# nsdumont/Semantic-Spiking-Neural-SLAM-2023

Hardware: AMD Instinct MI355X
Metric: sim-sec/wall-sec, SSP-SLAM ssp_dim=1015 10k PI neurons, 1/2/4/8 MI355X (higher is better)
Workload: dtype f32; 1 GPU; PathIntegration 2-D ssp_dim=1015 pi_n_neurons=10000/VCO (508 VCOs, 5080000 LIF neurons), configs[1]; eval_points_per_vco=4000, parallelism=1 GPU, build_cache=miss

## Files before the change

semantic-spiking-neural-slam-2023_amd/csrc/ssn_block.hpp:

```cpp
#pragma once
#include <type_traits>
#include "ssn_launch.hpp"

namespace ssn {

__device__ inline float wave_sum_dpp(float v) {
  int x;
#define SSN_DPP_ADD(ctrl, rmask)                                                                             \
  x = __builtin_amdgcn_update_dpp(0, __builtin_bit_cast(int, v), ctrl, rmask, 0xF, false);                    \
  v += __builtin_bit_cast(float, x);
  SSN_DPP_ADD(0xB1, 0xF)
  SSN_DPP_ADD(0x4E, 0xF)
  SSN_DPP_ADD(0x141, 0xF)
  SSN_DPP_ADD(0x140, 0xF)
  SSN_DPP_ADD(0x142, 0xA)
  SSN_DPP_ADD(0x143, 0xC)
#undef SSN_DPP_ADD
  return v;
}
__device__ inline float row_sum_dpp(float v) {
  int x;
#define SSN_DPP_ADD(ctrl)                                                                                    \
  x = __builtin_amdgcn_update_dpp(0, __builtin_bit_cast(int, v), ctrl, 0xF, 0xF, false);                      \
  v += __builtin_bit_cast(float, x);
// ... 124 lines not shown
  const f32x2 Wn = pk_fma_clamp01_vs_negv(spk, big, U);
  w = __builtin_elementwise_fma(spk, nu, Wn + nmt);
}
__device__ inline void lif_finish_silent(f32x2& w, f32x2 U, f32x2 nmt) {
  f32x2 Wn;
  asm("v_pk_mul_f32 %0, %1, -1.0 op_sel_hi:[1,0] clamp" : "=v"(Wn) : "v"(U));
  w = Wn + nmt;
}
__device__ inline f32x2 lif_input_part(f32x2 Jm1, f32x2& w, f32x2 W0, f32x2 em, const LifConstV3P& c, f32x2 big) {
  const f32x2 nmt = pk_sub_clamp01(w, (f32x2)(c.m1));
  const f32x2 U = __builtin_elementwise_fma(Jm1 + W0, em, -W0);
  const f32x2 spk = pk_mul_clamp01(U, big);
  f32x2 rc;
  rc.x = __builtin_amdgcn_rcpf(Jm1.x);
  rc.y = __builtin_amdgcn_rcpf(Jm1.y);
  f32x2 Wn, u, P, nu;
  asm("v_pk_fma_f32 %0, %2, %3, %4 neg_lo:[0,0,1] neg_hi:[0,0,1] clamp\n\t"
      "v_pk_mul_f32 %1, %4, %5"
      : "=&v"(Wn), "=v"(u)
      : "v"(spk), "s"(big), "v"(U), "v"(rc));
  asm("v_pk_fma_f32 %0, %1, %2, %3" : "=v"(P) : "v"(u), "v"((f32x2)(c.p2)), "s"((f32x2)(c.p1)));
  asm("v_pk_fma_f32 %0, %1, %2, %3" : "=v"(P) : "v"(u), "v"(P), "s"((f32x2)(c.p0)));
  asm("v_pk_fma_f32 %0, %1, %2, %3 clamp" : "=v"(nu) : "v"(u), "v"(P), "s"((f32x2)(c.ktau_ref)));
  w = __builtin_elementwise_fma(spk, nu, Wn + nmt);
  return spk;
}
__device__ inline float lif_word_in(float s, float K) { return __builtin_fmaf(-s, s < 0.0f ? K : 1.0f, 1.0f); }
__device__ inline float lif_word_out(float w, float K) { return (1.0f - w) * (w > 1.0f ? 1.0f / K : 1.0f); }

__device__ inline float bits_f(unsigned int x) { return __builtin_bit_cast(float, x); }
__device__ inline unsigned int f_bits(float x) { return __builtin_bit_cast(unsigned int, x); }

#ifdef SSN_BLOCK_STAMPS
__device__ unsigned long long g_block_stamps[9];
inline hipError_t read_block_stamps(unsigned long long* out, int reset) {
  hipError_t e = hipMemcpyFromSymbol(out, HIP_SYMBOL(g_block_stamps), sizeof(unsigned long long) * 9);
  if (e == hipSuccess && reset) {
    const unsigned long long z[9] = {0, 0, 0, 0, 0, 0, 0, 0, 0};
    e = hipMemcpyToSymbol(HIP_SYMBOL(g_block_stamps), z, sizeof z);
  }
  return e;
}
#define SSN_BSTAMP(var)                                                                          \
  do {                                                                                           \
    __builtin_amdgcn_sched_barrier(0);                                                           \
    asm volatile("s_memtime %0\n\ts_waitcnt lgkmcnt(0)" : "=s"(var) :: "memory");                \
    __builtin_amdgcn_sched_barrier(0);                                                           \
  } while (0)
#define SSN_BSTAMP_ADD(i, a, b) bst[i] += (b) - (a)
#else
#define SSN_BSTAMP(var) do {} while (0)
#define SSN_BSTAMP_ADD(i, a, b) do {} while (0)
#endif

#ifndef SSN_BLOCK_SKIP
#define SSN_BLOCK_SKIP 0
#endif
#ifndef SSN_BLOCK_PIPE
#define SSN_BLOCK_PIPE 1
#endif
#ifndef SSN_BLOCK_HOIST_A
#define SSN_BLOCK_HOIST_A 2
#endif
#ifndef SSN_BLOCK_HOIST_B
#define SSN_BLOCK_HOIST_B 4
#endif
#ifndef SSN_BLOCK_HOIST_C
#define SSN_BLOCK_HOIST_C 2
#endif
struct BlockHoist { int a, b, c; };
constexpr BlockHoist block_hoist(bool pipe, int tpb, int ng) {
  if (!pipe || SSN_BLOCK_SKIP != 0) return {0, 0, 0};
  const int room = tpb <= 512 && ng >= 10 ? ng : 0;
  const int c = SSN_BLOCK_HOIST_C >= 2 && room >= 2 ? 2 : 0;
  int b = SSN_BLOCK_HOIST_B < room - c ? SSN_BLOCK_HOIST_B : room - c;
  int a_ = SSN_BLOCK_HOIST_A < room - c - b ? SSN_BLOCK_HOIST_A : room - c - b;
  return {a_, b, c};
}

template <typename T, int DIN, int DOUT, int NPT, int TPB, int LDSW, int SPLIT = 0, int TAP = 0>
__global__ __launch_bounds__(TPB) void k_ens_block(BlockArgs<T> a) {
  static_assert(!(SPLIT && TAP), "the split kernel has no tapped form");
  constexpr bool ENC_LDS = LDSW == DIN;
  static_assert(LDSW == 0 || LDSW == DIN, "LDSW");
  extern __shared__ __align__(16) unsigned char ssn_block_dyn[];
  T* const e_lds = reinterpret_cast<T*>(ssn_block_dyn);
  constexpr bool F32 = sizeof(T) == 4;
  constexpr int PK = F32 ? 2 : 1;
  constexpr int NG = NPT / PK;
  static_assert(NPT % PK == 0, "f32 variants handle neuron pairs");
  constexpr bool PIPE = F32 && NG >= 5 && SSN_BLOCK_PIPE != 0;
  constexpr BlockHoist HO = block_hoist(PIPE, TPB, NG);
  constexpr int HC = HO.c, HA = HO.a, HB = HO.b, HT = HC + HA + HB;
  using G = typename std::conditional<F32, f32x2, T>::type;
  constexpr int DP = DOUT <= 4 ? 4 : 8;
  static_assert(!SPLIT || (sizeof(T) == 4 && DOUT <= 4), "split ensembles: f32, at most four decoded rows");
  const int P = SPLIT ? a.P : 1;
  const int k = P > 1 ? (int)blockIdx.x / P : (int)blockIdx.x;
  const int member = P > 1 ? (int)blockIdx.x - k * P : 0;
  const int noff = member * a.n_member;
  const int n_loc = P > 1 ? max(0, min(a.n_member, a.n_pad - noff)) : a.n_pad;
  const int tid = threadIdx.x;
  const int nthr = NG == 1 ? (int)blockDim.x : TPB;
  const int lane = tid & 63, wave = tid >> 6;
  const size_t row = (size_t)a.n_pad;
  const T* __restrict__ enc = a.enc + (size_t)k * DIN * row + noff;
  const T* __restrict__ bias = a.bias + (size_t)k * row + noff;
  T* __restrict__ Sp = a.S + (size_t)k * row + noff;
  const NeuronParams<T> np = a.np;
  const LifMath<T> lm(np);
  const int* tcol = nullptr;
  if constexpr (TAP != 0) {
    const int tslot = a.tap_slot[k];
    if (tslot >= 0) tcol = a.tap_col + (size_t)tslot * row;
// ... 18 lines not shown
    return reinterpret_cast<const G*>(e_lds + lrow[d] + g * nthr * PK);
  };
#pragma unroll
  for (int g = 0; g < NG; ++g) {
    const int i0 = (g * nthr + tid) * PK;
    const bool in = i0 < n_loc;
    const int ii = in ? i0 : 0;
    const T msk = in ? T(1) : T(0);
    auto ld = [&](const T* p) -> G { if constexpr (F32) return *reinterpret_cast<const f32x2*>(p) * msk; else return *p * msk; };
#pragma unroll
    for (int d = 0; d < DIN; ++d) {
      const G ev = ld(enc + d * row + ii);
      if constexpr (ENC_LDS) *reinterpret_cast<G*>(e_lds + d * cap + i0) = ev; else e[g][d] = ev;
    }
    b[g] = ld(bias + ii);
    s[g] = ld(Sp + ii);
    if constexpr (F32) {
      b[g] = b[g] - 1.0f;
      s[g] = (f32x2){lif_word_in(s[g].x, lcK), lif_word_in(s[g].y, lcK)};
    }
    if (a.dec_neuron_major) {
      const T* dp = a.dec + ((size_t)k * row + noff + ii) * DP;
#pragma unroll
      for (int r = 0; r < DOUT; ++r) {
        if constexpr (F32) dc[g][r] = (f32x2){dp[r], dp[DP + r]} * msk; else dc[g][r] = dp[r] * msk;
      }
    } else {
      const T* dp = a.dec + (size_t)k * DOUT * row + noff + ii;
#pragma unroll
      for (int r = 0; r < DOUT; ++r) dc[g][r] = ld(dp + r * row);
    }
  }

  constexpr int CH = 32;
  constexpr int XP = 4;
  constexpr int RW = DOUT <= 4 ? 64 : 128;
  __shared__ __align__(16) T red[2][RW];
  __shared__ __align__(16) T xs[CH][XP];
  __shared__ T os[CH][DOUT];
  __shared__ int s_dst[DOUT];
  __shared__ int s_out[DOUT];
  for (int i = tid; i < 2 * RW; i += nthr) (&red[0][0])[i] = T(0);
  if (tid < DOUT) { s_dst[tid] = a.didx[(long long)k * DOUT + tid]; s_out[tid] = a.rowout[(long long)k * DOUT + tid] ? 1 : 0; }
  const T* __restrict__ xbase = a.xrows + (size_t)a.row0 * a.n_sig + a.x_off + (long long)k * DIN;

  T fs[F32 ? 1 : DOUT], la[F32 ? 1 : DOUT], lb[F32 ? 1 : DOUT], tot[F32 ? 1 : DOUT];
  float F0 = 0.0f, F1 = 0.0f, la0 = 0.0f, lb0 = 0.0f, la1 = 0.0f, lb1 = 0.0f, v0 = 0.0f, v1 = 0.0f;
  T xa[DIN];
  int xr[DIN];
#pragma unroll
  for (int d = 0; d < DIN; ++d) {
    xr[d] = a.xrow[(long long)k * DIN + d];
    xa[d] = xr[d] >= 0 ? a.xalpha[(long long)k * DIN + d] : T(0);
  }
  if constexpr (F32) {
    const int r0 = lane >> 4;
    if (r0 < DOUT) {
      const long long i = (long long)k * DOUT + r0;
      const int st = a.lp_state[i];
      if (st >= 0) { F0 = a.sig[st]; la0 = a.lp_a[i]; lb0 = a.lp_b[i]; }
    }
    if (DOUT > 4) {
      const long long i = (long long)k * DOUT + 4;
      const int st = a.lp_state[i];
      if (st >= 0) { F1 = a.sig[st]; la1 = a.lp_a[i]; lb1 = a.lp_b[i]; }
    }
  } else {
#pragma unroll
    for (int r = 0; r < DOUT; ++r) {
      const long long i = (long long)k * DOUT + r;
      const int st = a.lp_state[i];
      fs[r] = st >= 0 ? a.sig[st] : T(0);
      la[r] = st >= 0 ? a.lp_a[i] : T(0);
      lb[r] = st >= 0 ? a.lp_b[i] : T(0);
// ... 13 lines not shown
  G en[ILE][LDSW > 0 ? LDSW : 1];
  if constexpr (ENC_LDS) {
#pragma unroll
    for (int u = 0; u < ILE; ++u)
#pragma unroll
      for (int d = 0; d < LDSW; ++d) en[u][d] = *lds_group(d, u);
  }
#ifdef SSN_BLOCK_STAMPS
  unsigned long long bst[6] = {0, 0, 0, 0, 0, 0}, bt0 = 0, bt1 = 0, bt2 = 0, bt3 = 0, bt4 = 0, bt5 = 0, bt6 = 0, bm0 = 0, br0 = 0;
  asm volatile("s_memtime %0\n\ts_memrealtime %1\n\ts_waitcnt lgkmcnt(0)" : "=s"(bm0), "=s"(br0) :: "memory");
#endif
  unsigned int n_slots = 0, n_silent = 0;
  T x[DIN];
  int xl[DIN];
#pragma unroll
  for (int d = 0; d < DIN; ++d) xl[d] = __builtin_amdgcn_readfirstlane((xr[d] & 3) << 4);
  auto assemble_x = [&](const float4 xv) {
    const float xin[4] = {xv.x, xv.y, xv.z, xv.w};
    float f1 = 0.0f;
    if constexpr (DOUT > 4) f1 = bits_f(__builtin_amdgcn_readlane(f_bits(F1), 0));
#pragma unroll
    for (int d = 0; d < DIN; ++d) {
      const float f0 = bits_f(__builtin_amdgcn_readlane(f_bits(F0), xl[d]));
      float st = f0;
      if constexpr (DOUT > 4) st = xr[d] >= 4 ? f1 : f0;
      x[d] = __builtin_fmaf(xa[d], st, xin[d]);
    }
  };
  f32x2 W0h[HT > 0 ? HT : 1], emh[HT > 0 ? HT : 1];
  if constexpr (HT > 0) {
#pragma unroll
    for (int g = 0; g < HT; ++g) lif_state_part(s[g], lc, W0h[g], emh[g]);
  }
  for (int j0 = 0; j0 < a.B; j0 += CH) {
    const int cn = min(CH, a.B - j0);
    __syncthreads();
    if (j0 > 0 && member == 0) {
      for (int i = tid; i < CH * DOUT; i += nthr) {
        const int jj = i / DOUT, r = i - jj * DOUT;
        if (s_out[r]) a.bsig[(size_t)(a.row0 + j0 - CH + jj) * a.n_sig + s_dst[r]] = os[jj][r];
      }
    }
    for (int i = tid; i < cn * DIN; i += nthr) {
      const int jj = i / DIN, d = i - jj * DIN;
      xs[jj][d] = xbase[(size_t)(j0 + jj) * a.n_sig + d];
    }
    __syncthreads();
    if constexpr (PIPE) {
      assemble_x(*(const float4*)xs[0]);
    }

    for (int jj = 0; jj < cn; ++jj) {
      SSN_BSTAMP(bt0);
      if constexpr (SPLIT != 0) {
        if (P > 1 && wave == 0 && (lane & 15) == 0) {
          unsigned int* const rst = a.xslots + (size_t)k * 64 + (size_t)((j0 + jj + 1) % 3) * ((size_t)a.K * 64) + member * 4 + (lane >> 4);
          const unsigned int sent = BLOCK_XCHG_SENTINEL;
          asm volatile("global_store_dword %0, %1, off sc0 sc1" :: "v"(rst), "v"(sent) : "memory");
        }
      }
      if constexpr (PIPE) {
      } else if constexpr (F32) {
        assemble_x(*(const float4*)xs[jj]);
      } else {
        T xin[XP];
        *(double2*)xin = *(const double2*)xs[jj]; *(double2*)(xin + 2) = *(const double2*)(xs[jj] + 2);
#pragma unroll
        for (int d = 0; d < DIN; ++d) {
          T st = T(0);
#pragma unroll
          for (int r = 0; r < DOUT; ++r) st = xr[d] == r ? fs[r] : st;
          x[d] = xr[d] >= 0 ? xin[d] + xa[d] * st : xin[d];
        }
      }
      SSN_BSTAMP(bt1);
      G accg[DOUT];
#pragma unroll
      for (int r = 0; r < DOUT; ++r) accg[r] = G(0);
      constexpr int IL = ILE;
#pragma unroll
      for (int g0 = 0; g0 < NG; g0 += IL) {
        G J[IL], spk[IL];
#pragma unroll
        for (int u = 0; u < IL; ++u) {
          const int g = g0 + u < NG ? g0 + u : NG - 1;
          J[u] = b[g];
#pragma unroll
          for (int d = 0; d < DIN; ++d) {
            if constexpr (ENC_LDS) J[u] += en[u][d] * x[d];
            else J[u] += e[g][d] * x[d];
          }
        }
        if constexpr (ENC_LDS) {
#pragma unroll
          for (int u = 0; u < IL; ++u) {
            if (g0 + u >= NG) continue;
            asm volatile("" : "+v"(J[u]));
            const int gn = g0 + IL + u < NG ? g0 + IL + u : (g0 + IL + u) % IL;
#pragma unroll
// ... 82 lines not shown
          if constexpr (TAP != 0) {
            if (tcol) {
              const int i0 = (g * nthr + tid) * PK;
              T* const trow = a.bsig + (size_t)(a.row0 + j0 + jj) * a.n_sig;
              if (i0 < n_loc) {
                if constexpr (F32) {
                  const int2 d = *reinterpret_cast<const int2*>(tcol + i0);
                  const f32x2 val = spk[u] * a.tap_amp;
                  if (d.x >= 0) trow[d.x] = val.x;
                  if (d.y >= 0) trow[d.y] = val.y;
                } else {
                  const int d = tcol[i0];
                  if (d >= 0) trow[d] = spk[u] * a.tap_amp;
                }
              }
            }
          }
          if constexpr (F32 && SSN_BLOCK_SKIP == 1) continue;
#pragma unroll
          for (int r = 0; r < DOUT; ++r) {
            if constexpr (F32) accg[r] = __builtin_elementwise_fma(spk[u], dc[g][r], accg[r]);
            else accg[r] = fma(spk[u], dc[g][r], accg[r]);
          }
        }
        }
#ifndef SSN_BLOCK_NO_SCHED_BARRIER
        if constexpr (F32) __builtin_amdgcn_sched_barrier(0);
#endif
      }
      const int par = jj & 1;
      SSN_BSTAMP(bt2);
      if constexpr (F32) {
        float4 xnx = {0.0f, 0.0f, 0.0f, 0.0f};
        if constexpr (PIPE) xnx = *(const float4*)xs[jj + 1 < cn ? jj + 1 : jj];
        (void)xnx;
        float acc[DOUT];
#pragma unroll
        for (int r = 0; r < DOUT; ++r) acc[r] = accg[r].x + accg[r].y;
        if constexpr (DOUT >= 4) {
          const auto p01 = __builtin_amdgcn_permlane32_swap(f_bits(acc[0]), f_bits(acc[1]), false, false);
          const auto p23 = __builtin_amdgcn_permlane32_swap(f_bits(acc[2]), f_bits(acc[3]), false, false);
          const float s01 = bits_f(p01[0]) + bits_f(p01[1]);
          const float s23 = bits_f(p23[0]) + bits_f(p23[1]);
          const auto q = __builtin_amdgcn_permlane16_swap(f_bits(s01), f_bits(s23), false, false);
          float t4 = bits_f(q[0]) + bits_f(q[1]);
          t4 = row_sum_dpp(t4);
          if constexpr (DOUT == 5) {
            const float w4 = wave_sum_dpp(acc[4]);
            if (wslot >= 0) red[par][wslot] = lane == 63 ? w4 : t4;
          } else {
            if (wslot >= 0) red[par][wslot] = t4;
          }
        } else {
          wave_sum_dpp_n<DOUT>(acc);
          if (lane == 63) {
#pragma unroll
            for (int r = 0; r < DOUT; ++r) red[par][r * 16 + wave] = acc[r];
          }
        }
        if constexpr (HA > 0) {
          __builtin_amdgcn_sched_barrier(0);
#pragma unroll
          for (int g = HC; g < HC + HA; ++g) lif_state_part(s[g], lc, W0h[g], emh[g]);
          __builtin_amdgcn_sched_barrier(0);
        }
        SSN_BSTAMP(bt3);
        __syncthreads();
// ... 38 lines not shown
          if (P > 1) {
            const int tq = j0 + jj;
            unsigned int* const xb = a.xslots + (size_t)k * 64;
            const size_t bstride = (size_t)a.K * 64;
            if (wave == 0 && (lane & 15) == 0) {
              unsigned int* const pub = xb + (size_t)(tq % 3) * bstride + member * 4 + (lane >> 4);
              const unsigned int val = f_bits(v0);
              asm volatile("s_waitcnt vmcnt(0)\n\tglobal_store_dword %0, %1, off sc0 sc1" :: "v"(pub), "v"(val) : "memory");
            }
            const unsigned int* const src = xb + (size_t)(tq % 3) * bstride + (lane & 15) * 4 + (lane >> 4);
            const bool mine = (lane & 15) < P;
            unsigned int got = 0, spins = 0;
            while (true) {
              if (mine) asm volatile("global_load_dword %0, %1, off sc0 sc1\n\ts_waitcnt vmcnt(0)" : "=v"(got) : "v"(src) : "memory");
              if (!__any(mine && got == BLOCK_XCHG_SENTINEL)) break;
              if (++spins > (1u << 20)) { if (lane == 0) *a.xerr = 1; break; }
            }
            v0 = row_sum_dpp(mine ? bits_f(got) : 0.0f);
          }
        }
        F0 = __builtin_fmaf(la0, F0, lb0 * v0);
        if constexpr (HC > 0) {
          __builtin_amdgcn_sched_barrier(0);
#pragma unroll
          for (int g = 0; g < HC; ++g) W0h[g] = pk_clamp01(s[g]);
          __builtin_amdgcn_sched_barrier(0);
        }
        if constexpr (DOUT > 4) {
          if constexpr (PIPE) v1 = row_sum_dpp(v1); else v1 = row_sum_dpp(red[par][64 + lane]);
          F1 = __builtin_fmaf(la1, F1, lb1 * v1);
        }
        if constexpr (PIPE) assemble_x(xnx);
        if (wave == 0 && member == 0) {
          if ((lane & 15) == 0 && (lane >> 4) < DOUT) os[jj][lane >> 4] = v0;
          if (DOUT > 4 && lane == 0) os[jj][4] = v1;
        }
        SSN_BSTAMP(bt6);
        SSN_BSTAMP_ADD(0, bt0, bt1); SSN_BSTAMP_ADD(1, bt1, bt2); SSN_BSTAMP_ADD(2, bt2, bt3); SSN_BSTAMP_ADD(3, bt3, bt4);
        SSN_BSTAMP_ADD(4, bt4, bt6); SSN_BSTAMP_ADD(5, bt4, bt5);
      } else {
        T acc[DOUT];
#pragma unroll
        for (int r = 0; r < DOUT; ++r) acc[r] = accg[r];
        wave_sum_dpp_n<DOUT>(acc);
        if (lane == 63) {
#pragma unroll
          for (int r = 0; r < DOUT; ++r) red[par][r * 16 + wave] = acc[r];
        }
        __syncthreads();
#pragma unroll
        for (int r = 0; r < DOUT; ++r) {
          T t = T(0);
#pragma unroll
          for (int w = 0; w < 16; ++w) t += red[par][r * 16 + w];
          tot[r] = t;
        }
#pragma unroll
        for (int r = 0; r < DOUT; ++r) fs[r] = la[r] * fs[r] + lb[r] * tot[r];
        if (tid < DOUT) {
          T v = T(0);
#pragma unroll
          for (int r = 0; r < DOUT; ++r) v = tid == r ? tot[r] : v;
          os[jj][tid] = v;
        }
      }
    }
  }
#ifdef SSN_BLOCK_STAMPS
  if constexpr (F32) {
    unsigned long long bm1, br1;
    asm volatile("s_memtime %0\n\ts_memrealtime %1\n\ts_waitcnt lgkmcnt(0)" : "=s"(bm1), "=s"(br1) :: "memory");
    if (lane == 0) {
      for (int i = 0; i < 5; ++i) atomicAdd(&g_block_stamps[i], bst[i]);
      atomicAdd(&g_block_stamps[8], bst[5]);
      atomicAdd(&g_block_stamps[5], (unsigned long long)a.B);
      if (k == 0 && wave == 0) { atomicAdd(&g_block_stamps[6], bm1 - bm0); atomicAdd(&g_block_stamps[7], br1 - br0); }
    }
  }
#endif
  if constexpr (F32 && SSN_BLOCK_SKIP != 0) {
    if (lane == 0 && a.slot_stats) {
      atomicAdd(a.slot_stats, (unsigned long long)n_slots);
      atomicAdd(a.slot_stats + 1, (unsigned long long)n_silent);
    }
  }
  __syncthreads();
  if (member == 0) {
    const int j0 = (a.B - 1) / CH * CH, cn = a.B - j0;
    for (int i = tid; i < cn * DOUT; i += nthr) {
      const int jj = i / DOUT, r = i - jj * DOUT;
      if (s_out[r]) a.bsig[(size_t)(a.row0 + j0 + jj) * a.n_sig + s_dst[r]] = os[jj][r];
    }
  }

  int tid2 = tid;
  asm volatile("" : "+v"(tid2));
#pragma unroll
  for (int g = 0; g < NG; ++g) {
    const int i0 = (g * nthr + tid2) * PK;
    if constexpr (F32) s[g] = (f32x2){lif_word_out(s[g].x, lcK), lif_word_out(s[g].y, lcK)};
    if (i0 < n_loc) *reinterpret_cast<G*>(Sp + i0) = s[g];
  }
  if constexpr (TAP != 0) {
    if (tcol && a.B > 0) {
      const T* const lrow = a.bsig + (size_t)(a.row0 + a.B - 1) * a.n_sig;
#pragma unroll
      for (int g = 0; g < NG; ++g) {
        const int i0 = (g * nthr + tid2) * PK;
        if (i0 >= n_loc) continue;
#pragma unroll
        for (int c = 0; c < PK; ++c) {
          const int d = tcol[i0 + c];
          if (d >= 0) a.sig_w[d] = lrow[d];
        }
      }
    }
  }
  if (a.B > 0 && member == 0) {
    if constexpr (F32) {
      if (wave == 0 && (lane & 15) == 0 && (lane >> 4) < DOUT) {
        const int r = lane >> 4;
        a.sig_w[s_dst[r]] = v0;
        const int st = a.lp_state[(long long)k * DOUT + r];
        if (st >= 0) a.sig_w[st] = F0;
      }
      if (DOUT > 4 && tid == 0) {
        a.sig_w[s_dst[4]] = v1;
        const int st = a.lp_state[(long long)k * DOUT + 4];
        if (st >= 0) a.sig_w[st] = F1;
      }
    } else if (tid < DOUT) {
      T v = T(0), f = T(0);
#pragma unroll
      for (int r = 0; r < DOUT; ++r) { v = tid == r ? tot[r] : v; f = tid == r ? fs[r] : f; }
      a.sig_w[s_dst[tid]] = v;
      const int st = a.lp_state[(long long)k * DOUT + tid];
      if (st >= 0) a.sig_w[st] = f;
    }
  }
}

constexpr int BLOCK_LDS_BYTES = 160 * 1024, BLOCK_STATIC_LDS = 2560;

template <typename T, int DIN, int DOUT, int NPT, int TPB, int LDSW, int SPLIT, int TAP = 0>
static hipError_t launch_block_variant_s(hipStream_t s, const BlockArgs<T>& a) {
  const int lds = LDSW * a.threads * NPT * (int)sizeof(T);
  static std::atomic<uint64_t> configured{0};
  if (LDSW > 0) {
    hipError_t e = set_max_dynamic_lds_once(reinterpret_cast<const void*>(&k_ens_block<T, DIN, DOUT, NPT, TPB, LDSW, SPLIT, TAP>),
                                            BLOCK_LDS_BYTES - BLOCK_STATIC_LDS, configured);
    if (e != hipSuccess) return e;
  }
  hipLaunchKernelGGL((k_ens_block<T, DIN, DOUT, NPT, TPB, LDSW, SPLIT, TAP>), dim3((unsigned)(a.K * (SPLIT ? a.P : 1))), dim3((unsigned)a.threads), lds, s, a);
  return hipGetLastError();
}
template <typename T, int DIN, int DOUT, int NPT, int TPB, int LDSW>
static hipError_t launch_block_variant(hipStream_t s, const BlockArgs<T>& a) {
  if (a.P > 1) {
    if constexpr (sizeof(T) == 4 && DOUT <= 4) return launch_block_variant_s<T, DIN, DOUT, NPT, TPB, LDSW, 1>(s, a);
    else return hipErrorInvalidValue;
  }
  if (a.tap_slot) {
    if constexpr (SSN_BLOCK_SKIP == 0) return launch_block_variant_s<T, DIN, DOUT, NPT, TPB, LDSW, 0, 1>(s, a);
    else return hipErrorInvalidValue;
  }
  return launch_block_variant_s<T, DIN, DOUT, NPT, TPB, LDSW, 0>(s, a);
}

struct BlockVariant { int tpb, npt, ldsw; };
template <typename T> struct BlockVariants;
template <> struct BlockVariants<float> {
  static constexpr int N = 7;
  static constexpr BlockVariant v[N] = {{1024, 2, 0}, {1024, 4, 0}, {512, 6, 0}, {1024, 6, 0}, {512, 10, 0}, {512, 20, 3}, {768, 14, 3}};
};
template <> struct BlockVariants<double> {
  static constexpr int N = 3;
  static constexpr BlockVariant v[N] = {{1024, 1, 0}, {1024, 2, 0}, {1024, 4, 0}};
};

template <typename T, int DIN, int DOUT>
static hipError_t launch_block_npt(hipStream_t s, const BlockArgs<T>& a) {
  const int key = (a.tpb * 100 + a.npt) * 8 + a.enc_lds;
  switch (key) {
#define SSN_CASE(TPB, N, L) case (TPB * 100 + N) * 8 + L: return launch_block_variant<T, DIN, DOUT, N, TPB, L>(s, a);
    SSN_CASE(1024, 2, 0) SSN_CASE(1024, 4, 0)
#undef SSN_CASE
#define SSN_CASE(TPB, N, L) case (TPB * 100 + N) * 8 + L: if constexpr (sizeof(T) == 8) return launch_block_variant<T, DIN, DOUT, N, TPB, L>(s, a); else return hipErrorInvalidValue;
    SSN_CASE(1024, 1, 0)
#undef SSN_CASE
#define SSN_CASE(TPB, N, L) case (TPB * 100 + N) * 8 + L: if constexpr (sizeof(T) == 4) return launch_block_variant<T, DIN, DOUT, N, TPB, L>(s, a); else return hipErrorInvalidValue;
    SSN_CASE(1024, 6, 0) SSN_CASE(512, 6, 0) SSN_CASE(512, 10, 0) SSN_CASE(512, 20, 3) SSN_CASE(768, 14, 3)
#undef SSN_CASE
    default: return hipErrorInvalidValue;
  }
}

template <typename T>
bool ens_block_supported(int din, int dout, int n, const int want[3], int* threads, int* tpb, int* npt, int* enc_lds) {
  if (!(din == 3 && dout >= 3 && dout <= 5)) return false;
  const int want_tpb = want[0], want_npt = want[1], want_lds = want[2];
  const int pk = sizeof(T) == 4 ? 2 : 1;
  for (int i = 0; i < BlockVariants<T>::N; ++i) {
    const BlockVariant v = BlockVariants<T>::v[i];
    if (want_tpb && (v.tpb != want_tpb || v.npt != want_npt || v.ldsw != want_lds)) continue;
    int th = v.tpb;
    if (v.npt == pk && n < th * pk) th = std::max(64, ((n + pk - 1) / pk + 63) / 64 * 64);
    if ((int64_t)th * v.npt < n) continue;
    if ((int64_t)v.ldsw * th * v.npt * (int64_t)sizeof(T) > BLOCK_LDS_BYTES - BLOCK_STATIC_LDS) continue;
    *threads = th; *tpb = v.tpb; *npt = v.npt; *enc_lds = v.ldsw;
    return true;
  }
  return false;
}

template <typename T>
hipError_t launch_ens_block(hipStream_t s, const BlockArgs<T>& a) {
  if (a.din == 3 && a.dout == 5) return launch_block_npt<T, 3, 5>(s, a);
  if (a.din == 3 && a.dout == 4) return launch_block_npt<T, 3, 4>(s, a);
  if (a.din == 3 && a.dout == 3) return launch_block_npt<T, 3, 3>(s, a);
  return hipErrorInvalidValue;
}

}
```

semantic-spiking-neural-slam-2023_amd/csrc/ssn_host.hip:

```cpp
#include <hip/hip_runtime.h>
#include <dlfcn.h>
#include <algorithm>
#include <climits>
#include <cmath>
#include <cstdarg>
#include <cstdio>
#include <cstdlib>
#include <cstring>
#include <memory>
#include <mutex>
#include <map>
#include <set>
#include <string>
#include <thread>
#include <vector>

#include "../../include/ssn.h"
#include "ssn_launch.hpp"

namespace {

__global__ void k_set_block(ssn::StepCtx* ctx, long long block_start) { ctx->block_start = block_start; }
__global__ void k_advance(ssn::StepCtx* ctx, long long n) { ctx->step += n; }

// ... 29 lines not shown
  do {                                \
    int rc__ = (expr);                \
    if (rc__ != SSN_OK) return rc__;  \
  } while (0)

struct Buf {
  void* d = nullptr;
  int64_t count = 0;
  int kind = 0;
  int64_t rows = 1, cols = 0, ld = 0;
  bool shaped = false;
  bool keep = false;
  std::vector<double> host;
  int dec_K = 0, dec_dout = 0, dec_n = 0, dec_DP = 0;
  int packed = 0;
  int partner = -1;
  bool transposed = false;
  int64_t ldt = 0;
  std::shared_ptr<std::vector<int32_t>> perm;
  int perm_rows = 1;
};

enum ItemType { IT_PROGRAM = 0, IT_ENS, IT_MATVEC, IT_NEURONS, IT_PES, IT_VOJA, IT_MATVEC_ORDERED, IT_FINISH, IT_SPMV, IT_DFT, IT_VECOPS, IT_GRID_LHS, IT_GRID_GEMM, IT_ARGMAX_PART, IT_ROUND,
                IT_GRID_DOT,
                IT_MATVEC_NEURONS,
                IT_NONE };

#define SSN_PLAN_KNOBS(X)                                                                                                                          \
  X(PRESENT, debug_plan, "SSN_DEBUG_PLAN", false, "print the plan to stderr at ssn_create (and per-item times after a profile = 2 run)")          \
  X(INT, debug_deps, "SSN_DEBUG_DEPS", UNSET, "first of four pipelined rounds whose instances are printed with what they wait for")                \
  X(INT, ens_sweeps, "SSN_ENS_SWEEPS", UNSET, "256-thread sweeps per workgroup of an ensemble array (clamped to what the array has)")            \
  X(OFF0, small_ens, "SSN_SMALL_ENS", true, "a wave per ensemble for arrays of many small 1-D ensembles (RK_ENS_SMALL)")                          \
  X(INT3, block_variant, "SSN_BLOCK_VARIANT", Int3(), "tpb,npt,lds of the whole-block kernel variant to use")                                     \
  X(INT, block_split, "SSN_BLOCK_SPLIT", UNSET, "member workgroups per ensemble of the split whole-block kernel (1, 2, 4 or 8; others ignored)")  \
  X(INT, block_split_cus, "SSN_BLOCK_SPLIT_CUS", UNSET, "CU count the split is sized for (tests: pretend the GPU is smaller / larger)")           \
  X(ON1, block_sort, "SSN_BLOCK_SORT", false, "whole-block kernel: neurons in slot order (only pays with a SSN_BLOCK_SKIP build)")               \
  X(PRESENT, dft_no_inplace, "SSN_DFT_NO_INPLACE", false, "Bluestein transforms never in place")                                                  \
  X(INT, spmv_max_chunks, "SSN_SPMV_MAX_CHUNKS", 64, "most chunks of a segmented spike list per sparse decode (at least 1)")                     \
  X(LL, grid_min_mb, "SSN_GRID_MIN_MB", 64, "smallest clean-up table (MB) whose similarities come from the factored grid as an MFMA product")     \
  X(LL, grid_dot_min_mb, "SSN_GRID_DOT_MIN_MB", 16, "smallest clean-up table (MB) that goes through its factor tables as bodies of the round grid") \
  X(INT, grid_split, "SSN_GRID_SPLIT", UNSET, "K-split of the grid product (clamped to 1..8)")                                                    \
  X(INT, matvec_r1_max, "SSN_MATVEC_R1_MAX", 4096, "tallest matrix that runs four rows per workgroup in a round (taller: sixteen)")              \
  X(REAL, cost_pes, "SSN_COST_PES", 2.0, "balancer: fraction of its matrix a PES update is priced at")                                            \
  X(REAL, cost_voja, "SSN_COST_VOJA", 0.2, "balancer: fraction of its matrix a Voja update is priced at")                                         \
  X(REAL, lat_dft, "SSN_LAT_DFT", 9.0, "balancer: latency of a transform body (us)")                                                              \
  X(REAL, lat_solo, "SSN_LAT_SOLO", 3.0, "balancer: latency of a gate / argmax body (us)")                                                        \
  X(OFF0, pes_fold, "SSN_PES_FOLD", true, "fold the filter of a PES rule's activities into the rule's body")                                      \
  X(ON1, phased_pes_fold, "SSN_PHASED_PES_FOLD", false, "... also in neuron-sharded plans")                                                       \
  X(OFF0, fuse_neurons, "SSN_FUSE_NEURONS", true, "neuron update of a dense population in the epilogue of its encoder product")                   \
  X(INT, fuse_min_rows, "SSN_FUSE_MIN_ROWS", 4097, "smallest population that is fused so (tests lower it)")                                       \
  X(OFF0, solo_chains, "SSN_SOLO_CHAINS", true, "serial chains of single-workgroup operators (RK_SOLO)")                                          \
  X(OFF0, phased_solo, "SSN_PHASED_SOLO", true, "... in neuron-sharded plans")                                                                    \
  X(ON1, solo_dft, "SSN_SOLO_DFT", false, "transforms as members of serial chains (measured slower)")                                             \
  X(REAL, solo_cap_us, "SSN_SOLO_CAP_US", 16.0, "longest serial chain in estimated microseconds")                                                 \
  X(LL, solo_max_len, "SSN_SOLO_MAX_LEN", 2048, "longest glue operator (elements) a single workgroup takes")                                      \
  X(OFF0, round_interleave, "SSN_ROUND_INTERLEAVE", true, "interleaved dispatch of a round's big grids behind its latency-bound head")            \
  X(OFF0, head_prio, "SSN_HEAD_PRIO", true, "raised wave priority for the head blocks of a round")                                                \
  X(PRESENT, phase2_sequential, "SSN_PHASE2_SEQUENTIAL", false, "sharded: phase 1 of a timestep and phase 0 of the next as two sets of rounds")   \
  X(INT, cycle_steps, "SSN_CYCLE_STEPS", 16, "sharded: timesteps pipelined over the exchange (2..64; 0 or 1: off)")                               \
  X(PRESENT, no_batch_reorder, "SSN_NO_BATCH_REORDER", false, "time-batched stages keep the builder's operator order")                            \
  X(PRESENT, no_zero_skip, "SSN_NO_ZERO_SKIP", false, "time-batched products are multiplied out even when their whole input is zero")

struct PlanOptions {
  struct Int3 { int v[3] = {0, 0, 0}; };
  static constexpr int UNSET = INT_MIN;
  enum Kind { K_PRESENT, K_OFF0, K_ON1, K_INT, K_LL, K_REAL, K_INT3 };
// ... 3244 lines not shown
    HIPCHK(hipSetDevice(device));
    if (phased) return fail(SSN_EINVAL, "a neuron-sharded model is stepped with ssn_run_phase (the caller exchanges between the phases)");
    if (n < 0) return fail(SSN_EINVAL, "negative step count");
    if (n == 0) return SSN_OK;
    int n_dom = 0;
    for (auto& it : items) n_dom += it.dominant ? 1 : 0;
    if (profile == 2 && (fused_block || core_empty)) profile = 1;
    Timing tm;
    tm.level = profile;
    if (profile) {
      const size_t per_step = profile == 2 ? items.size() + (round_mode ? launch_list.size() : 0) : (size_t)std::max(1, n_dom);
      const size_t need = fused_block ? (size_t)(2 * (n / std::max(1, block) + 2)) : (size_t)(2 * n * (int)per_step);
      if (need > 400000) return fail(SSN_EINVAL, "profile run too long (%lld steps): at most 200000 timed launches", (long long)n);
      while (ev_pool.size() < need) {
        hipEvent_t ev;
        HIPCHK(hipEventCreate(&ev));
        ev_pool.push_back(ev);
      }
    }
    HIPCHK(hipEventRecord(ev_run0, stream));
    int64_t done = 0;
    while (done < n) {
      const int64_t B = bsig ? std::min<int64_t>(block, n - done) : (n - done);
      const int64_t step0 = steps_done + done;
      if (bsig) {
        hipLaunchKernelGGL(k_set_block, dim3(1), dim3(1), 0, stream, d_ctx, (long long)step0);
        HIPCHK(hipGetLastError());
        HIPCHK(run_batch(pre_ops, (int)B, step0));
      }
      if (fused_defer) HIPCHK(ssn::launch_ens_finish<T>(stream, fin_begin));
      if (fused_block) {
        const bool timed = profile && B == block && tm.used + 2 <= ev_pool.size();
        blk.B = (int)B;
        if (blk.P > 1)
          HIPCHK(hipMemsetD32Async((hipDeviceptr_t)blk.xslots, (int)ssn::BLOCK_XCHG_SENTINEL, (size_t)3 * blk.K * 64, stream));
        if (timed) HIPCHK(hipEventRecord(ev_pool[tm.used], stream));
        HIPCHK(ssn::launch_ens_block<T>(stream, blk));
        if (timed) { HIPCHK(hipEventRecord(ev_pool[tm.used + 1], stream)); tm.used += 2; }
        HIPCHK(advance_clock(B));
      } else if (core_empty) {
        HIPCHK(advance_clock(B));
      } else if (profile) {
        int64_t s = 0;
        if (profile == 2 && round_mode && !graph_list.empty())
          for (; s + steps_per_graph <= B; s += steps_per_graph) {
            HIPCHK(launch_seq(graph_list, &tm));
            HIPCHK(advance_clock(steps_per_graph));
          }
        for (; s < B; ++s) {
          HIPCHK(launch_seq(launch_list, &tm));
          if (fused_defer) HIPCHK(advance_clock(1));
        }
      } else {
        int64_t left = B;
        if (step_graph.exec)
          for (; left >= steps_per_graph; left -= steps_per_graph) HIPCHK(hipGraphLaunch(step_graph.exec, stream));
        if (left > 0) HIPCHK(launch_steps((int)left, true));
      }
      if (fused_defer) HIPCHK(ssn::launch_ens_finish<T>(stream, fin_flush));
      if (bsig) {
        HIPCHK(run_batch(post_ops, (int)B, step0));
        HIPCHK(hipMemcpyAsync(bsig, bsig + (size_t)B * n_sig, (size_t)n_sig * sizeof(T), hipMemcpyDeviceToDevice, stream));
      }
      done += B;
    }
    HIPCHK(hipEventRecord(ev_run1, stream));
// ... 346 lines not shown
```

semantic-spiking-neural-slam-2023_amd/csrc/ssn_launch.hpp:

```cpp
#pragma once
#include <hip/hip_runtime.h>
#include <stdint.h>
#include <atomic>

namespace ssn {

inline hipError_t set_max_dynamic_lds_once(const void* fn, int bytes, std::atomic<uint64_t>& done) {
  int dev = 0;
  hipError_t e = hipGetDevice(&dev);
  if (e != hipSuccess) return e;
  const uint64_t bit = 1ull << (dev & 63);
  if (done.load(std::memory_order_acquire) & bit) return hipSuccess;
  e = hipFuncSetAttribute(fn, hipFuncAttributeMaxDynamicSharedMemorySize, bytes);
  if (e == hipSuccess) done.fetch_or(bit, std::memory_order_release);
  return e;
}

template <typename T>
struct NeuronParams {
  int type;
  T dt, tau_rc, tau_ref, min_voltage;
};

struct StepCtx;
// ... 52 lines not shown
  const unsigned char* rowout;
  T* sig;
  T* bsig;
  long long n_sig;
  StepCtx* ctx;
  unsigned int* ticket;
  int K, P, dout, n_blocks;
  int mode;
  T* fstate;
  long long partials_stride;
  const int* lp_has;
};

template <typename T>
struct BlockArgs {
  const T* enc;
  const T* bias;
  const T* dec;
  T* S;
  const T* xrows;
  T* bsig;
  const T* sig;
  T* sig_w;
  const int* didx;
  const int* lp_state;
  const T* lp_a;
  const T* lp_b;
  const int* xrow;
  const T* xalpha;
  const unsigned char* rowout;
  long long n_sig, x_off;
  int K, n, n_pad, din, dout;
  int B;
  int row0;
  int threads, tpb, npt;
  int dec_neuron_major;
  int enc_lds;
  NeuronParams<T> np;
  int P;
  int n_member;
  unsigned int* xslots;
  int* xerr;
  unsigned long long* slot_stats;
  const int* tap_slot;
  const int* tap_col;
  T tap_amp;
};
constexpr unsigned int BLOCK_XCHG_SENTINEL = 0x7fc0deadu;
#ifndef SSN_BLOCK_IL
#define SSN_BLOCK_IL 2
#endif

struct DftArgs {
  const float* src;
  float* dst;
  const float2* tw;
  int N;
  int kind;
  int set;
  int nr;
  int radix[12];
  int M;
  const float2* chirp;
  const float2* fb;
  int inplace;
  int N1, N2;
  const float* g1;
  const float* g2;
};

constexpr int MAX_BATCH = 4;
template <typename T> struct MatvecArgs { const T* Wm; const T* src; T* dst; int rows, cols, ld, set; };
template <typename T> struct MatvecBatch { MatvecArgs<T> a[MAX_BATCH]; };
template <typename T> struct NeuronsArgs { NeuronParams<T> np; const T* J; T* out; T* V; T* R; int n; T amp; int* seg_list; int* seg_cnt; };
template <typename T> struct NeuronsBatch { NeuronsArgs<T> a[MAX_BATCH]; };
template <typename T> struct MatvecNeuronsArgs { MatvecArgs<T> mv; NeuronsArgs<T> nr; };
struct DftBatch { DftArgs a[MAX_BATCH]; };
template <typename T> struct SpmvArgs { const T* Wt; int ldt; const T* spikes; int n, rows; T* partial; int rows_pad, chunks; const int* list; const int* count;
                                       int seg; int seg_len; };
template <typename T> struct SpmvBatch { SpmvArgs<T> a[MAX_BATCH]; };
constexpr int MAX_ENS_BATCH = 2;
// ... 130 lines not shown
```

Measured before the change: 363.0 sim-sec/wall-sec.

## Size whole-block kernel I/O chunks dynamically from free LDS and batch input staging

Replaces the fixed 32-step LDS chunk for input rows and decoded outputs with a runtime chunk size, stored in dynamic LDS after the encoder area. The chunk is sized to fill the remaining LDS, up to the batch length. This cuts the number of per-chunk barrier, staging and writeback rounds in the time loop. The input staging loop is also unrolled so each thread issues several global loads before its LDS stores, and extra edge timestamps are added under the stamps build. The cost is a much larger dynamic LDS request, which can reduce occupancy, although the kernel runs one workgroup per ensemble.

```diff
diff --git a/semantic-spiking-neural-slam-2023_amd/csrc/ssn_block.hpp b/semantic-spiking-neural-slam-2023_amd/csrc/ssn_block.hpp
--- a/semantic-spiking-neural-slam-2023_amd/csrc/ssn_block.hpp
+++ b/semantic-spiking-neural-slam-2023_amd/csrc/ssn_block.hpp
@@ -180,11 +180,11 @@
 __device__ inline unsigned int f_bits(float x) { return __builtin_bit_cast(unsigned int, x); }
 
 #ifdef SSN_BLOCK_STAMPS
-__device__ unsigned long long g_block_stamps[9];
+__device__ unsigned long long g_block_stamps[12];
 inline hipError_t read_block_stamps(unsigned long long* out, int reset) {
-  hipError_t e = hipMemcpyFromSymbol(out, HIP_SYMBOL(g_block_stamps), sizeof(unsigned long long) * 9);
+  hipError_t e = hipMemcpyFromSymbol(out, HIP_SYMBOL(g_block_stamps), sizeof(unsigned long long) * 12);
   if (e == hipSuccess && reset) {
-    const unsigned long long z[9] = {0, 0, 0, 0, 0, 0, 0, 0, 0};
+    const unsigned long long z[12] = {0, 0, 0, 0, 0, 0, 0, 0, 0, 0, 0, 0};
     e = hipMemcpyToSymbol(HIP_SYMBOL(g_block_stamps), z, sizeof z);
   }
   return e;
@@ -228,6 +228,10 @@
 
 template <typename T, int DIN, int DOUT, int NPT, int TPB, int LDSW, int SPLIT = 0, int TAP = 0>
 __global__ __launch_bounds__(TPB) void k_ens_block(BlockArgs<T> a) {
+#ifdef SSN_BLOCK_STAMPS
+  unsigned long long be_entry = 0, be_last = 0, be_end = 0, bedge[2] = {0, 0};
+  SSN_BSTAMP(be_entry);
+#endif
   static_assert(!(SPLIT && TAP), "the split kernel has no tapped form");
   constexpr bool ENC_LDS = LDSW == DIN;
   static_assert(LDSW == 0 || LDSW == DIN, "LDSW");
@@ -312,14 +316,16 @@
     }
   }
 
-  constexpr int CH = 32;
-  constexpr int XP = 4;
+  constexpr int XP = BLOCK_XP;
   constexpr int RW = DOUT <= 4 ? 64 : 128;
   __shared__ __align__(16) T red[2][RW];
-  __shared__ __align__(16) T xs[CH][XP];
-  __shared__ T os[CH][DOUT];
   __shared__ int s_dst[DOUT];
   __shared__ int s_out[DOUT];
+  static_assert(sizeof(T) * 2 * RW + 2 * sizeof(int) * DOUT + 32 <= BLOCK_STATIC_LDS, "static LDS of k_ens_block (plus alignment) over its bound");
+  constexpr size_t ENC_BYTES = ENC_LDS ? sizeof(T) * DIN * cap : 0;
+  const int ch = a.ch;
+  T* const xs = reinterpret_cast<T*>(ssn_block_dyn + ENC_BYTES);
+  T* const os = xs + (size_t)ch * XP;
   for (int i = tid; i < 2 * RW; i += nthr) (&red[0][0])[i] = T(0);
   if (tid < DOUT) { s_dst[tid] = a.didx[(long long)k * DOUT + tid]; s_out[tid] = a.rowout[(long long)k * DOUT + tid] ? 1 : 0; }
   const T* __restrict__ xbase = a.xrows + (size_t)a.row0 * a.n_sig + a.x_off + (long long)k * DIN;
@@ -399,26 +405,44 @@
 #pragma unroll
     for (int g = 0; g < HT; ++g) lif_state_part(s[g], lc, W0h[g], emh[g]);
   }
-  for (int j0 = 0; j0 < a.B; j0 += CH) {
-    const int cn = min(CH, a.B - j0);
+  for (int j0 = 0; j0 < a.B; j0 += ch) {
+    const int cn = min(ch, a.B - j0);
     __syncthreads();
     if (j0 > 0 && member == 0) {
-      for (int i = tid; i < CH * DOUT; i += nthr) {
+      for (int i = tid; i < ch * DOUT; i += nthr) {
         const int jj = i / DOUT, r = i - jj * DOUT;
-        if (s_out[r]) a.bsig[(size_t)(a.row0 + j0 - CH + jj) * a.n_sig + s_dst[r]] = os[jj][r];
+        if (s_out[r]) a.bsig[(size_t)(a.row0 + j0 - ch + jj) * a.n_sig + s_dst[r]] = os[jj * DOUT + r];
       }
     }
-    for (int i = tid; i < cn * DIN; i += nthr) {
-      const int jj = i / DIN, d = i - jj * DIN;
-      xs[jj][d] = xbase[(size_t)(j0 + jj) * a.n_sig + d];
+    {
+      constexpr int SU = TPB <= 512 ? 8 : 4;
+      const int ne = cn * DIN;
+      for (int i0 = tid; i0 < ne; i0 += SU * nthr) {
+        T xv[SU];
+#pragma unroll
+        for (int u = 0; u < SU; ++u) {
+          const int i = min(i0 + u * nthr, ne - 1);
+          const int jj = i / DIN, d = i - jj * DIN;
+          xv[u] = xbase[(size_t)(j0 + jj) * a.n_sig + d];
+        }
+#pragma unroll
+        for (int u = 0; u < SU; ++u) {
+          const int i = i0 + u * nthr;
+          const int jj = i / DIN, d = i - jj * DIN;
+          if (i < ne) xs[jj * XP + d] = xv[u];
+        }
+      }
     }
     __syncthreads();
     if constexpr (PIPE) {
-      assemble_x(*(const float4*)xs[0]);
+      assemble_x(*(const float4*)xs);
     }
 
     for (int jj = 0; jj < cn; ++jj) {
       SSN_BSTAMP(bt0);
+#ifdef SSN_BLOCK_STAMPS
+      if (jj == 0) { if (j0 == 0) bedge[0] = bt0 - be_entry; else bedge[1] += bt0 - be_last; }
+#endif
       if constexpr (SPLIT != 0) {
         if (P > 1 && wave == 0 && (lane & 15) == 0) {
           unsigned int* const rst = a.xslots + (size_t)k * 64 + (size_t)((j0 + jj + 1) % 3) * ((size_t)a.K * 64) + member * 4 + (lane >> 4);
@@ -428,10 +452,10 @@
       }
       if constexpr (PIPE) {
       } else if constexpr (F32) {
-        assemble_x(*(const float4*)xs[jj]);
+        assemble_x(*(const float4*)(xs + jj * XP));
       } else {
         T xin[XP];
-        *(double2*)xin = *(const double2*)xs[jj]; *(double2*)(xin + 2) = *(const double2*)(xs[jj] + 2);
+        *(double2*)xin = *(const double2*)(xs + jj * XP); *(double2*)(xin + 2) = *(const double2*)(xs + jj * XP + 2);
 #pragma unroll
         for (int d = 0; d < DIN; ++d) {
           T st = T(0);
@@ -580,7 +604,7 @@
       SSN_BSTAMP(bt2);
       if constexpr (F32) {
         float4 xnx = {0.0f, 0.0f, 0.0f, 0.0f};
-        if constexpr (PIPE) xnx = *(const float4*)xs[jj + 1 < cn ? jj + 1 : jj];
+        if constexpr (PIPE) xnx = *(const float4*)(xs + (jj + 1 < cn ? jj + 1 : jj) * XP);
         (void)xnx;
         float acc[DOUT];
 #pragma unroll
@@ -685,10 +709,13 @@
         }
         if constexpr (PIPE) assemble_x(xnx);
         if (wave == 0 && member == 0) {
-          if ((lane & 15) == 0 && (lane >> 4) < DOUT) os[jj][lane >> 4] = v0;
-          if (DOUT > 4 && lane == 0) os[jj][4] = v1;
+          if ((lane & 15) == 0 && (lane >> 4) < DOUT) os[jj * DOUT + (lane >> 4)] = v0;
+          if (DOUT > 4 && lane == 0) os[jj * DOUT + 4] = v1;
         }
         SSN_BSTAMP(bt6);
+#ifdef SSN_BLOCK_STAMPS
+        be_last = bt6;
+#endif
         SSN_BSTAMP_ADD(0, bt0, bt1); SSN_BSTAMP_ADD(1, bt1, bt2); SSN_BSTAMP_ADD(2, bt2, bt3); SSN_BSTAMP_ADD(3, bt3, bt4);
         SSN_BSTAMP_ADD(4, bt4, bt6); SSN_BSTAMP_ADD(5, bt4, bt5);
       } else {
@@ -714,22 +741,14 @@
           T v = T(0);
 #pragma unroll
           for (int r = 0; r < DOUT; ++r) v = tid == r ? tot[r] : v;
-          os[jj][tid] = v;
+          os[jj * DOUT + tid] = v;
         }
       }
     }
   }
 #ifdef SSN_BLOCK_STAMPS
-  if constexpr (F32) {
-    unsigned long long bm1, br1;
-    asm volatile("s_memtime %0\n\ts_memrealtime %1\n\ts_waitcnt lgkmcnt(0)" : "=s"(bm1), "=s"(br1) :: "memory");
-    if (lane == 0) {
-      for (int i = 0; i < 5; ++i) atomicAdd(&g_block_stamps[i], bst[i]);
-      atomicAdd(&g_block_stamps[8], bst[5]);
-      atomicAdd(&g_block_stamps[5], (unsigned long long)a.B);
-      if (k == 0 && wave == 0) { atomicAdd(&g_block_stamps[6], bm1 - bm0); atomicAdd(&g_block_stamps[7], br1 - br0); }
-    }
-  }
+  unsigned long long bm1 = 0, br1 = 0;
+  if constexpr (F32) asm volatile("s_memtime %0\n\ts_memrealtime %1\n\ts_waitcnt lgkmcnt(0)" : "=s"(bm1), "=s"(br1) :: "memory");
 #endif
   if constexpr (F32 && SSN_BLOCK_SKIP != 0) {
     if (lane == 0 && a.slot_stats) {
@@ -739,10 +758,10 @@
   }
   __syncthreads();
   if (member == 0) {
-    const int j0 = (a.B - 1) / CH * CH, cn = a.B - j0;
+    const int j0 = (a.B - 1) / ch * ch, cn = a.B - j0;
     for (int i = tid; i < cn * DOUT; i += nthr) {
       const int jj = i / DOUT, r = i - jj * DOUT;
-      if (s_out[r]) a.bsig[(size_t)(a.row0 + j0 + jj) * a.n_sig + s_dst[r]] = os[jj][r];
+      if (s_out[r]) a.bsig[(size_t)(a.row0 + j0 + jj) * a.n_sig + s_dst[r]] = os[jj * DOUT + r];
     }
   }
 
@@ -791,20 +810,36 @@
       if (st >= 0) a.sig_w[st] = f;
     }
   }
-}
-
-constexpr int BLOCK_LDS_BYTES = 160 * 1024, BLOCK_STATIC_LDS = 2560;
+#ifdef SSN_BLOCK_STAMPS
+  if constexpr (F32) {
+    SSN_BSTAMP(be_end);
+    if (lane == 0) {
+      for (int i = 0; i < 5; ++i) atomicAdd(&g_block_stamps[i], bst[i]);
+      atomicAdd(&g_block_stamps[8], bst[5]);
+      atomicAdd(&g_block_stamps[5], (unsigned long long)a.B);
+      if (k == 0 && wave == 0) { atomicAdd(&g_block_stamps[6], bm1 - bm0); atomicAdd(&g_block_stamps[7], br1 - br0); }
+    }
+    if (tid == 0 && a.B > 0) {
+      atomicAdd(&g_block_stamps[9], bedge[0]);
+      atomicAdd(&g_block_stamps[10], bedge[1]);
+      atomicAdd(&g_block_stamps[11], be_end - be_last);
+    }
+  }
+#endif
+}
 
 template <typename T, int DIN, int DOUT, int NPT, int TPB, int LDSW, int SPLIT, int TAP = 0>
 static hipError_t launch_block_variant_s(hipStream_t s, const BlockArgs<T>& a) {
-  const int lds = LDSW * a.threads * NPT * (int)sizeof(T);
+  const long long enc = (long long)LDSW * a.threads * NPT * (long long)sizeof(T);
+  const long long lds = enc + (long long)a.ch * (BLOCK_XP + DOUT) * (long long)sizeof(T);
+  if (a.ch < 1 || lds > BLOCK_LDS_BYTES - BLOCK_STATIC_LDS) return hipErrorInvalidValue;
   static std::atomic<uint64_t> configured{0};
-  if (LDSW > 0) {
+  {
     hipError_t e = set_max_dynamic_lds_once(reinterpret_cast<const void*>(&k_ens_block<T, DIN, DOUT, NPT, TPB, LDSW, SPLIT, TAP>),
                                             BLOCK_LDS_BYTES - BLOCK_STATIC_LDS, configured);
     if (e != hipSuccess) return e;
   }
-  hipLaunchKernelGGL((k_ens_block<T, DIN, DOUT, NPT, TPB, LDSW, SPLIT, TAP>), dim3((unsigned)(a.K * (SPLIT ? a.P : 1))), dim3((unsigned)a.threads), lds, s, a);
+  hipLaunchKernelGGL((k_ens_block<T, DIN, DOUT, NPT, TPB, LDSW, SPLIT, TAP>), dim3((unsigned)(a.K * (SPLIT ? a.P : 1))), dim3((unsigned)a.threads), (size_t)lds, s, a);
   return hipGetLastError();
 }
 template <typename T, int DIN, int DOUT, int NPT, int TPB, int LDSW>
@@ -859,7 +894,7 @@
     int th = v.tpb;
     if (v.npt == pk && n < th * pk) th = std::max(64, ((n + pk - 1) / pk + 63) / 64 * 64);
     if ((int64_t)th * v.npt < n) continue;
-    if ((int64_t)v.ldsw * th * v.npt * (int64_t)sizeof(T) > BLOCK_LDS_BYTES - BLOCK_STATIC_LDS) continue;
+    if ((int64_t)v.ldsw * th * v.npt * (int64_t)sizeof(T) + (int64_t)BLOCK_MIN_CHUNK * (BLOCK_XP + dout) * (int64_t)sizeof(T) > BLOCK_LDS_BYTES - BLOCK_STATIC_LDS) continue;
     *threads = th; *tpb = v.tpb; *npt = v.npt; *enc_lds = v.ldsw;
     return true;
   }
diff --git a/semantic-spiking-neural-slam-2023_amd/csrc/ssn_host.hip b/semantic-spiking-neural-slam-2023_amd/csrc/ssn_host.hip
--- a/semantic-spiking-neural-slam-2023_amd/csrc/ssn_host.hip
+++ b/semantic-spiking-neural-slam-2023_amd/csrc/ssn_host.hip
@@ -85,6 +85,7 @@
   X(INT, ens_sweeps, "SSN_ENS_SWEEPS", UNSET, "256-thread sweeps per workgroup of an ensemble array (clamped to what the array has)")            \
   X(OFF0, small_ens, "SSN_SMALL_ENS", true, "a wave per ensemble for arrays of many small 1-D ensembles (RK_ENS_SMALL)")                          \
   X(INT3, block_variant, "SSN_BLOCK_VARIANT", Int3(), "tpb,npt,lds of the whole-block kernel variant to use")                                     \
+  X(INT, block_chunk, "SSN_BLOCK_CHUNK", UNSET, "most timesteps per LDS-staged I/O chunk of the whole-block kernel (at least 1; tests: multi-chunk launches)") \
   X(INT, block_split, "SSN_BLOCK_SPLIT", UNSET, "member workgroups per ensemble of the split whole-block kernel (1, 2, 4 or 8; others ignored)")  \
   X(INT, block_split_cus, "SSN_BLOCK_SPLIT_CUS", UNSET, "CU count the split is sized for (tests: pretend the GPU is smaller / larger)")           \
   X(ON1, block_sort, "SSN_BLOCK_SORT", false, "whole-block kernel: neurons in slot order (only pays with a SSN_BLOCK_SKIP build)")               \
@@ -3395,6 +3396,8 @@
       if (fused_block) {
         const bool timed = profile && B == block && tm.used + 2 <= ev_pool.size();
         blk.B = (int)B;
+        blk.ch = ssn::block_chunk_steps((int)B, blk.enc_lds * blk.threads * blk.npt * (int)sizeof(T), blk.dout, (int)sizeof(T),
+                                        opt.block_chunk == PlanOptions::UNSET ? 0 : std::max(1, opt.block_chunk));
         if (blk.P > 1)
           HIPCHK(hipMemsetD32Async((hipDeviceptr_t)blk.xslots, (int)ssn::BLOCK_XCHG_SENTINEL, (size_t)3 * blk.K * 64, stream));
         if (timed) HIPCHK(hipEventRecord(ev_pool[tm.used], stream));
diff --git a/semantic-spiking-neural-slam-2023_amd/csrc/ssn_launch.hpp b/semantic-spiking-neural-slam-2023_amd/csrc/ssn_launch.hpp
--- a/semantic-spiking-neural-slam-2023_amd/csrc/ssn_launch.hpp
+++ b/semantic-spiking-neural-slam-2023_amd/csrc/ssn_launch.hpp
@@ -108,6 +108,7 @@
   long long n_sig, x_off;
   int K, n, n_pad, din, dout;
   int B;
+  int ch;
   int row0;
   int threads, tpb, npt;
   int dec_neuron_major;
@@ -123,6 +124,15 @@
   T tap_amp;
 };
 constexpr unsigned int BLOCK_XCHG_SENTINEL = 0x7fc0deadu;
+constexpr int BLOCK_LDS_BYTES = 160 * 1024, BLOCK_STATIC_LDS = 2560;
+constexpr int BLOCK_XP = 4;
+constexpr int BLOCK_MIN_CHUNK = 32;
+inline int block_chunk_steps(int B, int enc_bytes, int dout, int elem, int cap) {
+  long long ch = ((long long)BLOCK_LDS_BYTES - BLOCK_STATIC_LDS - enc_bytes) / ((long long)(BLOCK_XP + dout) * elem);
+  if (ch > B) ch = B;
+  if (cap > 0 && ch > cap) ch = cap;
+  return ch < 1 ? 1 : (int)ch;
+}
 #ifndef SSN_BLOCK_IL
 #define SSN_BLOCK_IL 2
 #endif
```

Measured after the change: 360.4 sim-sec/wall-sec. Within noise of the previous version (-0.7%).
